# DecodeGenetics/graphtyper

Measured on AMD Instinct MI355X. Metric: aligned+genotyped reads/sec over 1 Mb graph region; VCF bit-identical, higher is better.
Workload: dtype u64/u32 integer (2-bit k-mer keys, byte compares, u32 atomics)

## Files before the change

graphtyper_amd/csrc/gtx_api.hip:

```cpp
#include <hip/hip_runtime.h>
#include <chrono>

#include <algorithm>
#include <cstdio>
#include <cstdlib>
#include <cstring>
#include <memory>
#include <string>

#include "gtx_ctx.hpp"

#include <map>
#include "gtx_devmem.hpp"
#include "gtx_switches.hpp"
#include "wave_hip.hpp"
#include "align_core.hpp"
#include "gtx_hbm_passes.hpp"
#include "score_core.hpp"
#include "score_replay.hpp"

namespace gtx
{
#ifdef GTX_PROF
constexpr uint64_t PROF_LOG_ENTRIES = 1u << 16, PROF_LOG_ENTRY = 16;
// ... 225 lines not shown
    gtx_read_meta next_meta = meta[base];
    for (uint32_t read = base; read < end; ++read)
    {
      gtx_read_meta const m = next_meta;
      if (read + 1 < end)
        next_meta = meta[read + 1];
      uint32_t const len = m.l_qseq;
      uint8_t const * read_seq = seq + static_cast<uint64_t>(read) * seq_stride;
      if (prefetch)
      {
        if (4 * lane < seq_stride)
          seq_words[lane] = next_word;
        WaveHip::lds_sync();
        if (read + 1 < end && 4 * lane < seq_stride)
          next_word = reinterpret_cast<uint32_t const *>(read_seq + seq_stride)[lane];
        read_seq = reinterpret_cast<uint8_t const *>(seq_words);
      }
      bool const too_short = len < 2 * K - 1, too_long = len > AlignCfg::MAX_READ;
      bool const rev = needs_reverse(m, force_both != 0);
      for (uint32_t orient = 0; orient < 2; ++orient)
      {
        uint32_t * rec = records + (static_cast<uint64_t>(read) * 2 + orient) * rec_words;
        if (too_short || too_long || (orient == 1 && !rev))
        {
          if (lane == 0)
          {
            rec[0] = too_long ? (static_cast<uint32_t>(GTX_ST_RECORD_OVERFLOW) << 16) : 0u;
            rec[1] = len << 16;
          }
          continue;
        }
        if (queue_all || !express_one<WaveHip>(g, ix, ws, read_seq, len, orient == 1, rec, rec_words))
        {
          if (lane == 0)
            pending[n_pending] = read * 2 + orient;
          ++n_pending;
        }
      }
    }
    if (n_pending)
    {
      WaveHip::lds_sync();
      uint32_t const at = wave_claim(queue_count, n_pending);
      for (uint32_t k = lane; k < n_pending; k += 64)
        queue[at + k] = pending[k];
      WaveHip::lds_sync();
    }
  }
#ifdef GTX_PROF
  WaveHip::lds_sync();
  if (threadIdx.x < 16)
    atomicAdd(g.prof + threadIdx.x, ws.prof_acc[threadIdx.x]);
#endif
}

template <class E4>
__device__ __forceinline__ void express4_pass(GraphView const & g, IndexView const & ix, uint8_t const * __restrict__ seq, uint32_t seq_stride,
                                              gtx_read_meta const * __restrict__ meta, uint32_t n_reads, uint32_t * __restrict__ records,
                                              uint32_t rec_words, uint32_t force_both, uint32_t * task_counter,
                                              uint32_t * __restrict__ queue, uint32_t * queue_count, uint32_t queue_all)
{
  __shared__ Express4Workspace<E4> ws;
  __shared__ uint8_t pending[2 * TASK_CHUNK];
  static_assert(2 * TASK_CHUNK <= 256, "pending[] holds task offsets as bytes");
  uint32_t const lane = threadIdx.x & 63u;
  for (;;)
  {
    uint32_t const base = wave_claim(task_counter, TASK_CHUNK);
    if (base >= n_reads)
      break;
    uint32_t const end = base + TASK_CHUNK < n_reads ? base + TASK_CHUNK : n_reads;
    uint32_t n_pending = 0;
    for (uint32_t first = base; first < end; first += 4)
    {
      uint32_t const n_valid = end - first < 4 ? end - first : 4;
      uint32_t const gi = lane >> 4;
      bool rev = false;
      if (gi < n_valid)
      {
        gtx_read_meta const m = meta[first + gi];
        uint32_t const len = m.l_qseq;
        rev = needs_reverse(m, force_both != 0) && len >= 2 * K - 1 && len <= AlignCfg::MAX_READ;
        if (!rev && (lane & 15u) == 0)
        {
          uint32_t * rec = records + (static_cast<uint64_t>(first + gi) * 2 + 1) * rec_words;
          rec[0] = len > AlignCfg::MAX_READ ? (static_cast<uint32_t>(GTX_ST_RECORD_OVERFLOW) << 16) : 0u;
          rec[1] = len << 16;
        }
      }
      unsigned long long const REV = __ballot(rev);
      uint32_t const fwd_mask = express4<WaveHip, E4>(g, ix, ws, seq, seq_stride, meta, first, n_valid, records, rec_words, queue_all != 0);
      for (uint32_t k = 0; k < n_valid; ++k)
      {
        if ((fwd_mask >> k) & 1u)
        {
          if (lane == 0)
            pending[n_pending] = static_cast<uint8_t>((first + k - base) * 2);
          ++n_pending;
        }
        if ((REV >> (16 * k)) & 1ull)
        {
          if (lane == 0)
            pending[n_pending] = static_cast<uint8_t>((first + k - base) * 2 + 1);
          ++n_pending;
        }
      }
    }
    if (n_pending)
    {
      WaveHip::lds_sync();
      uint32_t const at = wave_claim(queue_count, n_pending);
      for (uint32_t k = lane; k < n_pending; k += 64)
        queue[at + k] = base * 2 + pending[k];
      WaveHip::lds_sync();
    }
  }
}

#define GTX_EXPRESS4_ARGS                                                                                                          \
  GraphView g, IndexView ix, uint8_t const *__restrict__ seq, uint32_t seq_stride, gtx_read_meta const *__restrict__ meta,         \
    uint32_t n_reads, uint32_t *__restrict__ records, uint32_t rec_words, uint32_t force_both, uint32_t *task_counter,             \
    uint32_t *__restrict__ queue, uint32_t *queue_count, uint32_t queue_all

#ifndef GTX_LEAN_WAVES
#define GTX_LEAN_WAVES 4
#endif
__global__ __launch_bounds__(64) __attribute__((amdgpu_waves_per_eu(GTX_LEAN_WAVES))) void gtx_align_express4_kernel(GTX_EXPRESS4_ARGS)
{
  express4_pass<Express4Lean>(g, ix, seq, seq_stride, meta, n_reads, records, rec_words, force_both, task_counter, queue, queue_count,
                              queue_all);
}

#ifndef GTX_WIDE_WAVES
#define GTX_WIDE_WAVES 4
#endif
__global__ __launch_bounds__(64) __attribute__((amdgpu_waves_per_eu(GTX_WIDE_WAVES))) void gtx_align_express4_wide_kernel(GTX_EXPRESS4_ARGS)
{
  express4_pass<Express4Wide>(g, ix, seq, seq_stride, meta, n_reads, records, rec_words, force_both, task_counter, queue, queue_count,
                              queue_all);
}

template <uint32_t WAVES, bool DENSE, uint32_t NK = AlignCfg::KC, bool META_LDS = true>
__device__ __forceinline__ void hinted_pass(GraphView const & g, IndexView const & ix, uint8_t const * __restrict__ seq, uint32_t seq_stride,
                                            gtx_read_meta const * __restrict__ meta, uint32_t n_reads, uint32_t * __restrict__ records,
                                            uint32_t rec_words, uint32_t force_both, uint32_t * __restrict__ queue1, uint32_t * __restrict__ queue2,
                                            unsigned long long * queue_counts ,
                                            uint32_t decline_all, uint8_t * __restrict__ task_flags, uint32_t * __restrict__ compact,
                                            unsigned long long * __restrict__ var_mask)
{
  constexpr uint32_t ROW_BYTES = HintGeom<NK>::ROW_BYTES, ROW_VEC = ROW_BYTES / 16, META_WORDS = sizeof(gtx_read_meta) / 4;
  constexpr uint32_t ROW_PITCH = NK == AlignCfg::KC ? ROW_VEC : ROW_VEC + 1;
  __shared__ uint4_t s_seq[WAVES][64 * ROW_PITCH];
  __shared__ uint32_t s_meta[META_LDS ? WAVES : 1][META_LDS ? 64 * META_WORDS : 1];
  auto s_count = [&](uint32_t q, uint32_t w) -> uint32_t & { return reinterpret_cast<uint32_t *>(&s_seq[w][0])[q]; };
  auto s_base = [&](uint32_t q) -> uint32_t & { return reinterpret_cast<uint32_t *>(&s_seq[0][0])[2 + q]; };
  static_assert(sizeof(gtx_read_meta) % 4 == 0, "meta records are staged word-wise");
  uint32_t const lane = threadIdx.x & 63u, wave = threadIdx.x >> 6;
  uint32_t const wave_first = blockIdx.x * blockDim.x + wave * 64u;
  uint32_t const read = wave_first + lane;
  bool const full = wave_first + 64u <= n_reads;
  bool const staged = full && seq_stride == ROW_BYTES && (reinterpret_cast<uintptr_t>(seq) & 15u) == 0;
  uint32_t own_meta[META_WORDS] = {};
  if constexpr (META_LDS)
  {
    if (full)
    {
      uint32_t const * src = reinterpret_cast<uint32_t const *>(meta + wave_first);
#pragma unroll
      for (uint32_t it = 0; it < META_WORDS; ++it)
        s_meta[wave][it * 64 + lane] = stream_load(src + it * 64 + lane);
    }
  }
  else if (read < n_reads)
  {
    uint32_t const * src = reinterpret_cast<uint32_t const *>(meta + read);
#pragma unroll
    for (uint32_t it = 0; it < META_WORDS; ++it)
      own_meta[it] = stream_load(src + it);
  }
  if (staged)
  {
    uint4_t const * src = reinterpret_cast<uint4_t const *>(seq + static_cast<uint64_t>(wave_first) * ROW_BYTES);
#pragma unroll
    for (uint32_t it = 0; it < ROW_VEC; ++it)
    {
      uint32_t const v = it * 64 + lane;
      s_seq[wave][ROW_PITCH == ROW_VEC ? v : (v / ROW_VEC) * ROW_PITCH + v % ROW_VEC] = stream_load(src + v);
    }
  }
  else if (read < n_reads)
  {
    uint8_t const * src = seq + static_cast<uint64_t>(read) * seq_stride;
    uint8_t * dst = reinterpret_cast<uint8_t *>(&s_seq[wave][lane * ROW_PITCH]);
#pragma unroll 1
    for (uint32_t k = 0; k < ROW_BYTES; ++k)
      dst[k] = k < seq_stride ? src[k] : static_cast<uint8_t>(0);
  }
  WaveHip::lds_sync();
  bool fwd = false, fwd2 = false, rev = false, staged_rec = false;
  uint32_t fwd_flag = 0;
  bool const compact_wave = compact != nullptr && task_flags != nullptr && full;
  static_assert(HINT_STAGE_WORDS == 16 && HINT_STAGE_WORDS * 4 <= ROW_BYTES, "a staged record is four 16-byte parts inside the read's row");
  if (read < n_reads)
  {
    gtx_read_meta m;
    if constexpr (!META_LDS)
    {
      uint32_t * mw = reinterpret_cast<uint32_t *>(&m);
#pragma unroll
      for (uint32_t k = 0; k < META_WORDS; ++k)
        mw[k] = own_meta[k];
    }
    else if (full)
    {
      uint32_t * mw = reinterpret_cast<uint32_t *>(&m);
#pragma unroll
      for (uint32_t k = 0; k < META_WORDS; ++k)
        mw[k] = s_meta[wave][lane * META_WORDS + k];
    }
    else
      m = meta[read];
    uint32_t const len = m.l_qseq;
    auto rec_at = [&]() -> uint32_t *
    {
      uint32_t r = read;
      GTX_PIN(r);
      return records + static_cast<uint64_t>(r) * 2 * rec_words;
    };
    bool const outside = len < 2 * K - 1 || len > AlignCfg::MAX_READ;
    rev = !outside && needs_reverse(m, force_both != 0);
    if (!rev && (m.flag & GTX_FLAG_FORWARD_ONLY) == 0)
    {
      uint32_t const h0 = len > AlignCfg::MAX_READ ? (static_cast<uint32_t>(GTX_ST_RECORD_OVERFLOW) << 16) : 0u;
      uint32_t * const rec = rec_at();
      if ((rec_words & 1u) == 0 && (reinterpret_cast<uintptr_t>(records) & 7u) == 0)
        *reinterpret_cast<uint2_t *>(rec + rec_words) = uint2_t{h0, len << 16};
      else
      {
        rec[rec_words] = h0;
        rec[rec_words + 1] = len << 16;
      }
    }
    if (outside)
    {
      uint32_t * const rec = rec_at();
      rec[0] = len > AlignCfg::MAX_READ ? (static_cast<uint32_t>(GTX_ST_RECORD_OVERFLOW) << 16) : 0u;
      rec[1] = len << 16;
    }
    else if ((decline_all & 1u) != 0)
      fwd = true;
    else
    {
      uint32_t * row = reinterpret_cast<uint32_t *>(&s_seq[wave][lane * ROW_PITCH]);
      bool const can_stage = (rec_words & 3u) == 0 && (reinterpret_cast<uintptr_t>(records) & 15u) == 0;
      uint32_t where;
      if constexpr (NK == AlignCfg::KC)
        where = hinted_one<DENSE>(g, ix, row, ROW_BYTES, m, rec_at, rec_words, can_stage ? row : nullptr);
      else
        where = hinted_long_one<NK>(g, ix, row, ROW_BYTES, m, rec_at(), rec_words, can_stage ? row : nullptr);
      fwd = where == 0;
      fwd2 = where == HINT_TO_GENERAL;
      staged_rec = where == 2;
      fwd_flag = (where == 0 || where == HINT_TO_GENERAL) ? 0u : ((where == 2 ? row[1] : rec_at()[1]) >> 31);
      if (compact_wave && staged_rec && (row[0] & 0xFFFFu) <= 1u && fwd_flag == 0)
      {
        staged_rec = false;
        fwd_flag = GTX_TASK_COMPACT;
      }
    }
    if ((decline_all & 4u) != 0 && fwd)
    {
      fwd = false;
      fwd2 = true;
    }
    if (task_flags)
    {
      bool const set_fwd = !fwd && !fwd2, set_rev = !rev;
      if (set_fwd && set_rev && (reinterpret_cast<uintptr_t>(task_flags) & 1u) == 0)
        *reinterpret_cast<uint16_t *>(task_flags + 2ull * read) = static_cast<uint16_t>(fwd_flag & 0xFFu);
      else
      {
        if (set_fwd)
          task_flags[2ull * read] = static_cast<uint8_t>(fwd_flag);
        if (set_rev)
          task_flags[2ull * read + 1] = 0;
      }
    }
  }
  if (var_mask)
  {
    unsigned long long const V = __ballot(read < n_reads && !fwd && !fwd2 && (fwd_flag & GTX_TASK_HAS_VARIANTS) != 0u);
    if (lane == 0 && wave_first < n_reads)
      var_mask[wave_first >> 6] = V;
  }
  if (compact_wave)
  {
    WaveHip::lds_sync();
    uint4_t * dst = reinterpret_cast<uint4_t *>(compact + static_cast<uint64_t>(wave_first) * GTX_COMPACT_WORDS);
#pragma unroll
    for (uint32_t k = 0; k < 2; ++k)
    {
      uint32_t const r = 32u * k + (lane >> 1);
      stream_store(dst + 64u * k + lane, s_seq[wave][r * ROW_PITCH + (lane & 1u)]);
    }
  }
  {
    unsigned long long const S = __ballot(staged_rec);
    if (S != 0)
    {
      uint32_t const part = lane & 3u;
#pragma unroll
      for (uint32_t round = 0; round < 4; ++round)
      {
        uint32_t const r = round * 16u + (lane >> 2);
        if ((S >> r) & 1ull)
        {
          uint4_t const v = s_seq[wave][r * ROW_PITCH + part];
          uint32_t const rd = wave_first + r;
          uint32_t * dst = records + static_cast<uint64_t>(rd) * 2 * rec_words;
          stream_store(reinterpret_cast<uint4_t *>(dst + 4 * part), v);
        }
      }
    }
  }
  unsigned long long const F = __ballot(fwd), R = __ballot(rev), F2 = __ballot(fwd2);
  if (lane == 0)
  {
    s_count(0, wave) = static_cast<uint32_t>(__builtin_popcountll(F));
    s_count(1, wave) = static_cast<uint32_t>(__builtin_popcountll(R) + __builtin_popcountll(F2));
  }
  __syncthreads();
  if (threadIdx.x == 0)
  {
    uint32_t total1 = 0, total2 = 0;
    for (uint32_t w = 0; w < WAVES; ++w)
    {
      total1 += s_count(0, w);
      total2 += s_count(1, w);
    }
    unsigned long long base = 0;
    if (total1 | total2)
      base = atomicAdd(queue_counts, (static_cast<unsigned long long>(total1) << 32) | total2);
    s_base(0) = static_cast<uint32_t>(base >> 32);
    s_base(1) = static_cast<uint32_t>(base);
  }
  __syncthreads();
  uint32_t off1 = s_base(0), off2 = s_base(1);
  for (uint32_t w = 0; w < WAVES; ++w)
    if (w < wave)
    {
      off1 += s_count(0, w);
      off2 += s_count(1, w);
    }
  if (fwd)
    queue1[off1 + static_cast<uint32_t>(__builtin_popcountll(F & ((1ull << lane) - 1ull)))] = read;
  if (rev)
    queue2[off2 + static_cast<uint32_t>(__builtin_popcountll(R & ((1ull << lane) - 1ull)))] = read * 2 + 1;
  if (fwd2)
    queue2[off2 + static_cast<uint32_t>(__builtin_popcountll(R) + __builtin_popcountll(F2 & ((1ull << lane) - 1ull)))] = read * 2;
}

#define GTX_HINTED_ARGS                                                                                                            \
  GraphView g, IndexView ix, uint8_t const *__restrict__ seq, uint32_t seq_stride, gtx_read_meta const *__restrict__ meta,         \
    uint32_t n_reads, uint32_t *__restrict__ records, uint32_t rec_words, uint32_t force_both, uint32_t *__restrict__ queue1,      \
    uint32_t *__restrict__ queue2, unsigned long long *queue_counts, uint32_t decline_all, uint8_t *__restrict__ task_flags,       \
    uint32_t *__restrict__ compact, unsigned long long *span, unsigned long long *__restrict__ var_mask
#define GTX_HINTED_PASS(W, ...)                                                                                                    \
  if (span && threadIdx.x == 0 && blockIdx.x == 0)                                                                                 \
    atomicMax(span, ~static_cast<unsigned long long>(wall_clock64()));                                                             \
  hinted_pass<W, __VA_ARGS__>(g, ix, seq, seq_stride, meta, n_reads, records, rec_words, force_both, queue1, queue2, queue_counts, decline_all, task_flags, compact, var_mask); \
  if (span && threadIdx.x == 0 && blockIdx.x + 1024u >= gridDim.x && ((blockIdx.x & 15u) == 15u || blockIdx.x + 1u == gridDim.x))   \
    atomicMax(span + 1, static_cast<unsigned long long>(wall_clock64()))

#ifndef GTX_HINT_VGPRS
#define GTX_HINT_VGPRS 72
#endif
#ifndef GTX_HINT_WAVES
#define GTX_HINT_WAVES 1
#endif
#ifndef GTX_HINT_PER_EU
#define GTX_HINT_PER_EU 7
#endif
#ifndef GTX_HINT_WAVES_LEAN
#define GTX_HINT_WAVES_LEAN 2
#endif
__global__ __launch_bounds__(64 * GTX_HINT_WAVES_LEAN) __attribute__((amdgpu_num_vgpr(GTX_HINT_VGPRS), amdgpu_waves_per_eu(GTX_HINT_PER_EU, GTX_HINT_PER_EU))) void gtx_align_hinted_kernel(GTX_HINTED_ARGS)
{
  GTX_HINTED_PASS(GTX_HINT_WAVES_LEAN, false, AlignCfg::KC, GTX_HINT_PER_EU <= 6);
}

#ifndef GTX_HINT_DENSE_WAVES
#define GTX_HINT_DENSE_WAVES 4
#endif
__global__ __launch_bounds__(64 * GTX_HINT_WAVES) __attribute__((amdgpu_waves_per_eu(GTX_HINT_DENSE_WAVES, GTX_HINT_DENSE_WAVES))) void gtx_align_hinted_dense_kernel(GTX_HINTED_ARGS)
{
  GTX_HINTED_PASS(GTX_HINT_WAVES, true);
}

__global__ __launch_bounds__(64 * GTX_HINT_WAVES) __attribute__((amdgpu_waves_per_eu(3, 3))) void gtx_align_hinted_long_kernel(GTX_HINTED_ARGS)
{
  GTX_HINTED_PASS(GTX_HINT_WAVES, false, 8);
}

constexpr uint32_t EXPRESS_GROUPS_PER_WAVE = 4, GENERAL_TASKS_PER_WAVE = 3;
template <class E4>
__device__ __forceinline__ void express4_queue_pass(GraphView const & g, IndexView const & ix, uint8_t const * __restrict__ seq,
                                                    uint32_t seq_stride, gtx_read_meta const * __restrict__ meta,
                                                    uint32_t * __restrict__ records, uint32_t rec_words, uint32_t * task_counter,
                                                    uint32_t const * __restrict__ queue1, uint32_t const * queue1_count,
                                                    uint32_t * __restrict__ queue2, uint32_t * queue2_count, uint32_t * handed_on,
                                                    uint32_t queue_all)
{
  __shared__ Express4Workspace<E4> ws;
  __shared__ uint32_t pending[TASK_CHUNK];
  uint32_t const lane = threadIdx.x & 63u;
  uint32_t const n = queue1_count[0];
  uint32_t const n_groups = (n + 3u) / 4u, G_all = gridDim.x;
  uint32_t const per_wave_goal = (queue_all >> 8) ? (queue_all >> 8) : EXPRESS_GROUPS_PER_WAVE;
  uint32_t const G_want = (n_groups + per_wave_goal - 1u) / per_wave_goal;
  uint32_t const G = G_want >= G_all ? G_all : G_want > 0u ? G_want : 1u;
  if (blockIdx.x >= G)
    return;
  uint32_t const own = n_groups / G <= 8u ? (n_groups / G) * 3u / 4u : 0u;
#ifdef GTX_PROF
  if (threadIdx.x < 16)
    ws.prof_acc[threadIdx.x] = 0;
  WaveHip::lds_sync();
#endif
  uint32_t n_pending = 0;
  auto flush = [&]()
  {
    if (n_pending)
    {
      WaveHip::lds_sync();
      uint32_t const at = wave_claim(queue2_count, n_pending);
      if (lane == 0)
        atomicAdd(handed_on, n_pending);
      for (uint32_t k = lane; k < n_pending; k += 64)
        queue2[at + k] = pending[k];
      WaveHip::lds_sync();
      n_pending = 0;
    }
  };
  uint32_t const per_visit = n_groups / G >= 128u ? 16u : n_groups / G >= 32u ? 4u : 1u;
  for (uint32_t i = 0, grp = 0, grp_end = 0;; ++i, ++grp)
  {
    if (i < own)
      grp = blockIdx.x + i * G;
    else if (i == own || grp == grp_end)
    {
      grp = own * G + wave_claim(task_counter, per_visit);
      grp_end = grp + per_visit;
    }
    if (grp >= n_groups)
      break;
    uint32_t const first = 4u * grp;
    uint32_t const n_valid = n - first < 4 ? n - first : 4;
    uint32_t const fwd_mask = express4<WaveHip, E4>(g, ix, ws, seq, seq_stride, meta, 0, n_valid, records, rec_words, (queue_all & 1u) != 0, queue1 + first);
    for (uint32_t k = 0; k < n_valid; ++k)
      if ((fwd_mask >> k) & 1u)
      {
        if (lane == 0)
          pending[n_pending] = queue1[first + k] * 2;
        ++n_pending;
      }
    if (n_pending + 4u > TASK_CHUNK)
      flush();
  }
  flush();
#ifdef GTX_PROF
  WaveHip::lds_sync();
  if (threadIdx.x < 16)
    atomicAdd(g.prof + 16 + threadIdx.x, ws.prof_acc[threadIdx.x]);
#endif
}

#define GTX_EXPRESS4Q_ARGS                                                                                                         \
  GraphView g, IndexView ix, uint8_t const *__restrict__ seq, uint32_t seq_stride, gtx_read_meta const *__restrict__ meta,         \
    uint32_t *__restrict__ records, uint32_t rec_words, uint32_t *task_counter, uint32_t const *__restrict__ queue1,               \
    uint32_t const *queue1_count, uint32_t *__restrict__ queue2, uint32_t *queue2_count, uint32_t *handed_on, uint32_t queue_all

__global__ __launch_bounds__(64) __attribute__((amdgpu_waves_per_eu(GTX_LEAN_WAVES))) void gtx_align_express4q_kernel(GTX_EXPRESS4Q_ARGS)
{
  express4_queue_pass<Express4Lean>(g, ix, seq, seq_stride, meta, records, rec_words, task_counter, queue1, queue1_count, queue2,
                                    queue2_count, handed_on, queue_all);
}

__global__ __launch_bounds__(64) __attribute__((amdgpu_waves_per_eu(GTX_WIDE_WAVES))) void gtx_align_express4q_wide_kernel(GTX_EXPRESS4Q_ARGS)
{
  express4_queue_pass<Express4Wide>(g, ix, seq, seq_stride, meta, records, rec_words, task_counter, queue1, queue1_count, queue2,
                                    queue2_count, handed_on, queue_all);
}

#ifndef GTX_GENERAL_WAVES
#define GTX_GENERAL_WAVES 5
#endif
__global__ __launch_bounds__(64) __attribute__((amdgpu_waves_per_eu(GTX_GENERAL_WAVES))) void gtx_align_kernel(GraphView g, IndexView ix, uint8_t const * __restrict__ seq,
                                                       uint32_t seq_stride, gtx_read_meta const * __restrict__ meta,
                                                       uint32_t * __restrict__ records, uint32_t rec_words,
                                                       uint32_t const * __restrict__ queue, uint32_t const * queue_count,
                                                       uint32_t * task_counter, uint32_t * __restrict__ big_tasks,
                                                       uint32_t big_task_cap, uint32_t * big_state, uint32_t force_big, uint32_t task_base,
                                                       uint32_t claim, uint32_t * forward_done)
{
  __shared__ AlignWorkspace ws;
#ifdef GTX_PROF
  if (threadIdx.x < 16)
    ws.prof_acc[threadIdx.x] = 0;
  WaveHip::lds_sync();
#endif
  uint32_t const queued = queue_count[0];
  uint32_t const per_wave_goal = (force_big >> 8) ? (force_big >> 8) : GENERAL_TASKS_PER_WAVE;
// ... 2282 lines not shown
```

graphtyper_amd/csrc/hinted.hpp:

```cpp
#pragma once
#include <type_traits>

#include "graph_dev.hpp"

namespace gtx
{
#ifdef GTX_EMU_NOTES
void hint_note(uint32_t code);
#define GTX_HINT_NOTE(code) hint_note(code)
#else
#define GTX_HINT_NOTE(code) ((void)0)
#endif

constexpr uint32_t HINT_MAX_READ = 160;
constexpr uint32_t HINT_WORDS = HINT_MAX_READ / 8;

GTX_DEV uint32_t hint_bswap(uint32_t v)
{
  return __builtin_bswap32(v);
}

GTX_DEV uint32_t nib_nonzero(uint32_t v)
{
  v |= v >> 1;
// ... 855 lines not shown
        {
          best = xa;
          mask = 0;
        }
        if (xa == best)
          mask |= 1u << a;
      }
    x0 = ((codes & 15u) != rc && rc != 15u) ? 1u : 0u;
    return best;
  };
  auto carried = [&](uint32_t km, uint32_t site) -> uint32_t
  {
    uint32_t set = (km >> HK_SET_SHIFT) & 255u;
    if (DENSE && hk_is_two(km))
    {
      uint32_t const s0 = km >> HK_SITE_SHIFT;
      if (site != s0 && site != s0 + 1u)
        return 4u;
      set = site == s0 ? (set & 15u) : (set >> 4);
      return (set & (set - 1u)) != 0 ? 4u : static_cast<uint32_t>(__builtin_ctz(set));
    }
    if ((km >> HK_SITE_SHIFT) != site || (set & (set - 1u)) != 0)
      return 4u;
    return set ? static_cast<uint32_t>(__builtin_ctz(set)) : (km >> HK_ALLELE_SHIFT) & 3u;
  };
  uint32_t head_site = 0, head_mask = 0;
  if (prs != 0 && !decided)
  {
    uint32_t const y = lo == 1 ? f1.y : lo == 2 ? f2.y : lo == 3 ? f3.y : f4.y;
    uint32_t const back = (y >> HINT_BACK_SHIFT) & 255u;
    uint32_t upto = hc_upto(h, lo) + hc_edge(h, lo);
    if ((y & 255u) == 0 || back < prs)
    {
      bool const on_site = (y & 255u) == 0;
      uint32_t const ps = on_site ? prs : prs - back - 1u;
      if (idx + ps == 0)
      {
        GTX_HINT_NOTE(11);
        return false;
      }
      uint32_t const q = idx + ps - 1u;
      uint32_t const yq = ix.pos_flags[q].y;
      uint2_t const tq = ix.tail_info[q];
      uint32_t const km = lo == 1 ? k1 : lo == 2 ? k2 : lo == 3 ? k3 : k4;
      uint32_t const only = on_site ? carried(km, tq.y) : 4u;
      if ((yq & 255u) != 1u || (tq.x & HINT_TAIL_OK) == 0 || (ps != 0 && ((yq >> HINT_BACK_SHIFT) & 255u) + 1u < ps) || (on_site && only >= 4u))
      {
        GTX_HINT_NOTE(11);
        return false;
      }
      uint32_t mask = 0, x0 = 0;
      uint32_t const best = site_choice(tq.x, plane_code_at(row, ps), only, mask, x0);
      upto = upto - x0 + best;
      head_site = tq.y;
      head_mask = mask;
    }
    uint32_t const head_len = prs + 1;
    uint32_t const budget = 2 + head_len / 11 < 7 ? 2 + head_len / 11 : 7;
    if (upto <= budget)
    {
      start = order_of(idx);
      rs = 0;
      mism += upto;
    }
    else
      head_mask = 0;
  }
  uint32_t end = order_of(idx + pre), re = pre;
  uint32_t tail_site = 0, tail_mask = 0;
  uint32_t tail_mask2 = 0;
  if (decided)
  {
    start = order_of(idx + two_rs);
    rs = two_rs;
    re = two_re;
    end = order_of(idx + two_re);
    mism = two_mism;
  }
  else if (pre != L - 1)
  {
    uint32_t const tail_len = L - pre;
    uint32_t const budget = 2 + tail_len / 11 < 7 ? 2 + tail_len / 11 : 7;
    uint32_t tail_end = DENSE ? order_of(idx + L - 1u) : 0u;
    uint32_t const y = hi + 1 == n_k ? y_end : hi == 0 ? f1.y : hi == 1 ? f2.y : hi == 2 ? f3.y : f4.y;
    uint32_t const room = y & 255u;
    uint32_t got = hc_all(h) - hc_upto(h, hi + 1);
    if (room < tail_len)
    {
      bool const on_site = room == 0;
      uint32_t const at = room;
      uint2_t ti = t_end;
      uint32_t only = 4u;
      bool ok = true;
      if (on_site)
      {
        uint32_t const q = idx + pre - 1u;
        ok = (ix.pos_flags[q].y & 255u) == 1u;
        ti = ix.tail_info[q];
        only = carried(hi == 0 ? k0 : hi == 1 ? k1 : hi == 2 ? k2 : hi == 3 ? k3 : k4, ti.y);
        ok = ok && only < 4u;
      }
      else if (hi + 1 != n_k)
        ti = ix.tail_info[idx + pre];
      uint32_t const next_len = (ti.x >> HINT_TAIL_NEXT_SHIFT) & 255u;
      if (!ok || (ti.x & HINT_TAIL_OK) == 0 || next_len < tail_len - at - 1)
      {
        bool walked = false;
        if constexpr (DENSE)
          if (!on_site && (ti.x & HINT_TAIL_NODE) != 0 && tail_len <= 64)
          {
            HintWalk const w = hint_tail_walk(g, ix, row, idx, pre, tail_len, at, ti.y, budget);
            if (w.status == 2)
            {
              GTX_HINT_NOTE(8);
              return HINT_TO_GENERAL;
            }
            if (w.status == 1)
            {
              walked = true;
              got = w.got;
              tail_end = w.end;
              tail_site = ti.y;
              tail_mask = w.mask1;
              tail_mask2 = w.mask2;
            }
          }
        if (!walked)
        {
          GTX_HINT_NOTE(8);
          return false;
        }
      }
      else
      {
        uint32_t mask = 0, x0 = 0;
        uint32_t const best = site_choice(ti.x, plane_code_at(row, pre + at), only, mask, x0);
        got = got - x0 + best;
        tail_site = ti.y;
        tail_mask = mask;
      }
    }
    if (got <= budget)
    {
      re = L - 1;
      mism += got;
      if constexpr (DENSE)
        end = tail_end;
      else
        end += tail_len - 1;
    }
    else
      tail_mask = tail_mask2 = 0;
  }
  uint32_t v0 = 0, v1 = 0, v2 = 0, v3 = 0, v4 = 0, v5 = 0;
  uint32_t nvar = 0;
  uint32_t last = 0xFFFFFFFFu;
  bool clash = false;
  auto append = [&](uint32_t entry)
  {
    if constexpr (DENSE)
    {
      bool found = false;
      auto meet = [&](uint32_t & v, uint32_t at)
      {
        if (at < nvar && (v >> 16) == (entry >> 16))
        {
          v &= entry | 0xFFFF0000u;
          clash = clash || (v & 0xFFFFu) == 0;
          found = true;
        }
      };
      meet(v0, 0);
      meet(v1, 1);
      meet(v2, 2);
      meet(v3, 3);
      meet(v4, 4);
      meet(v5, 5);
      if (!found)
      {
        v0 = nvar == 0 ? entry : v0;
        v1 = nvar == 1 ? entry : v1;
        v2 = nvar == 2 ? entry : v2;
        v3 = nvar == 3 ? entry : v3;
        v4 = nvar == 4 ? entry : v4;
        v5 = nvar == 5 ? entry : v5;
        ++nvar;
      }
    }
    else if ((entry >> 16) == (last >> 16))
    {
      last &= entry | 0xFFFF0000u;
      clash = clash || (last & 0xFFFFu) == 0;
      v0 = nvar == 1 ? last : v0;
      v1 = nvar == 2 ? last : v1;
      v2 = nvar == 3 ? last : v2;
      v3 = nvar == 4 ? last : v3;
      v4 = nvar == 5 ? last : v4;
      v5 = nvar == 6 ? last : v5;
    }
    else
    {
      v0 = nvar == 0 ? entry : v0;
      v1 = nvar == 1 ? entry : v1;
      v2 = nvar == 2 ? entry : v2;
      v3 = nvar == 3 ? entry : v3;
      v4 = nvar == 4 ? entry : v4;
      v5 = nvar == 5 ? entry : v5;
      ++nvar;
      last = entry;
    }
  };
  auto push = [&](uint32_t k, uint32_t km)
  {
    if (((run >> k) & 1u) && (km >> HK_SITE_SHIFT) != HINT_NO_SITE)
    {
      uint32_t const set = (km >> HK_SET_SHIFT) & 255u;
      if (DENSE && hk_is_two(km))
      {
        append(((km >> HK_SITE_SHIFT) << 16) | (set & 15u));
        append((((km >> HK_SITE_SHIFT) + 1u) << 16) | (set >> 4));
      }
      else
        append(((km >> HK_SITE_SHIFT) << 16) | (set ? set : 1u << ((km >> HK_ALLELE_SHIFT) & 3u)));
    }
  };
  if (tail_mask != 0)
    append((tail_site << 16) | tail_mask);
  if (tail_mask2 != 0)
    append(((tail_site + 1u) << 16) | tail_mask2);
  push(4, k4);
  push(3, k3);
  push(2, k2);
  push(1, k1);
  push(0, k0);
  if (head_mask != 0)
    append((head_site << 16) | head_mask);
  if (clash || nvar > 6 || 6 + 3 * nvar > rec_words)
  {
    GTX_HINT_NOTE(13);
    return false;
  }
  uint32_t np = 1, longest = re - rs + 1;
  if (par_start && rs == 0)
  {
    uint32_t const amb_lo = hc_get(lo == 1 ? h.k[1] : lo == 2 ? h.k[2] : lo == 3 ? h.k[3] : h.k[4], HC_AMB);
    uint2_t const f_lo = lo == 1 ? f1 : lo == 2 ? f2 : lo == 3 ? f3 : f4;
    bool two_chains = amb_lo != 0;
    if (!two_chains)
    {
      uint32_t const off = (f_lo.y >> HINT_SNPOFF_SHIFT) & 31u;
      if ((f_lo.x & HINT_ALT_OK) == 0 || off == K - 1)
      {
        GTX_HINT_NOTE(106);
        return HINT_TO_GENERAL;
      }
      two_chains = off != 0;
    }
    if (two_chains)
    {
      uint32_t const mm_run = mmk & run, km_hi = hi == 0 ? k0 : hi == 1 ? k1 : hi == 2 ? k2 : hi == 3 ? k3 : k4;
      auto plain = [&](uint32_t k, uint32_t km) { return ((run >> k) & 1u) == 0 || (km & ((3u << HK_ALLELE_SHIFT) | (255u << HK_SET_SHIFT))) == 0; };
      uint32_t alt_sites = 0;
      uint32_t const other = (plain(0, k0) ? 0u : 1u) | (plain(1, k1) ? 0u : 2u) | (plain(2, k2) ? 0u : 4u) | (plain(3, k3) ? 0u : 8u) | (plain(4, k4) ? 0u : 16u);
      if (other != 0)
      {
        uint32_t const k = static_cast<uint32_t>(__builtin_ctz(other));
        uint32_t const km = k == 0 ? k0 : k == 1 ? k1 : k == 2 ? k2 : k == 3 ? k3 : k4;
        uint32_t const yk = ix.pos_flags[idx + (K - 1) * k].y;
        bool ok = ix.hint_less == 0 && mm_run == 0 && pw == nullptr;
        ok = ok && (other & (other - 1u)) == 0 && ((km >> HK_SET_SHIFT) & 255u) == 0;
        alt_sites = (K - 1) * k + ((yk >> HINT_SNPOFF_SHIFT) & 31u) < pre ? 1u : 0u;
        if (!ok)
        {
          GTX_HINT_NOTE(107);
          return HINT_TO_GENERAL;
        }
      }
      bool const region_clean = hc_upto(h, hi + 1) == hc_upto(h, lo) + alt_sites;
      if (mm_run == (1u << hi) && hi + 1 > 4)
      {
        GTX_HINT_NOTE(108);
        return HINT_TO_GENERAL;
      }
      bool const last_only = mm_run == (1u << hi) && hc_edge(h, hi + 1) == 1 && ((km_hi >> HK_SET_SHIFT) & 255u) == 0;
      bool const twin = region_clean && (mm_run == 0 || last_only);
      if (pre == L - 1 || re != L - 1 || (twin && nvar > 1))
      {
        GTX_HINT_NOTE(109);
        return HINT_TO_GENERAL;
      }
      if (twin && mm_run == 0)
        np = 2;
      else if (twin)
        --mism;
    }
  }
  if (mism > 10)
  {
    np = 0;
    longest = 0;
  }
  uint32_t const path_words = 4 + 3 * nvar;
  if (2 + np * path_words > rec_words)
    return false;
  bool const to_stage = stage != nullptr && rec_words >= HINT_STAGE_WORDS && 2 + (np ? np : 1u) * path_words <= HINT_STAGE_WORDS;
  uint32_t * rec = to_stage ? stage : hint_rec_ptr(rec_at);
  if (to_stage)
  {
#pragma unroll
    for (uint32_t k = 2; k < HINT_STAGE_WORDS; ++k)
      rec[k] = 0u;
  }
  rec[0] = np;
  rec[1] = longest | (L << 16) | ((np && nvar) ? GTX_REC_HAS_VARIANTS : 0u);
  if (np)
  {
    rec[2] = start;
    rec[3] = end;
    rec[4] = rs | (re << 16);
    rec[5] = mism | (nvar << 16);
    auto put = [&](uint32_t k, uint32_t entry)
    {
      if (k < nvar)
      {
        rec[6 + 3 * k] = entry >> 16;
        rec[7 + 3 * k] = entry & 0xFFFFu;
        rec[8 + 3 * k] = 0u;
      }
    };
    put(0, v0);
    put(1, v1);
    put(2, v2);
    put(3, v3);
    put(4, v4);
    put(5, v5);
    if (np == 2)
      for (uint32_t k = 0; k < path_words; ++k)
        rec[2 + path_words + k] = rec[2 + k];
  }
  return to_stage ? 2u : 1u;
}

template <bool DENSE, class Row, class Rec>
GTX_DEV uint32_t hinted_one(GraphView const & g, IndexView const & ix, Row row, uint32_t seq_stride, gtx_read_meta const & m,
                            Rec rec, uint32_t rec_words, uint32_t * stage = nullptr)
{
  uint32_t const L = m.l_qseq;
  if (L < 2 * K - 1 || L > HINT_MAX_READ || m.pos < 0 || ix.n_hint == 0)
  {
    GTX_HINT_NOTE(9);
    return false;
  }
  if (static_cast<uint32_t>(m.pos) < ix.hint_first)
    return false;
  uint32_t const idx = static_cast<uint32_t>(m.pos) - ix.hint_first;
  if (idx >= ix.n_hint || L > ix.n_hint - idx)
    return false;
  uint32_t mm_main = 0xFFFFu;
  uint32_t where = hinted_on_path<DENSE>(g, ix, row, seq_stride, m, idx, static_cast<HintWindow const *>(nullptr), 0u, rec, rec_words, stage, mm_main);
  if constexpr (DENSE)
  {
    if (where == 0 && ix.n_win != 0 && mm_main != 0xFFFFu)
    {
      uint2_t const t0 = ix.tail_info[idx];
      if ((t0.x & HINT_TAIL_NODE) != 0)
      {
        uint32_t best = mm_main, best_at = 0, best_w = INVALID, tried = 0;
        uint32_t r = t0.y;
#pragma unroll 1
        for (uint32_t s = 0; s < 4 && r + 1 < g.n_ref; ++s, ++r)
        {
          uint32_t const off = g.ref_order[r] + g.ref_len[r] - (g.first_order + idx);
          if (off >= L)
            break;
          uint32_t const sw = ix.site_win[r], first = sw & 0xFFFFFFu, count = sw >> 24;
#pragma unroll 1
          for (uint32_t k = 0; k < count && tried < 8; ++k, ++tried)
          {
            uint32_t const at = ix.win_base + (first + k) * HINT_WIN_STRIDE + (HINT_WIN_BEFORE - off);
            uint32_t const mm = hint_mm_linear(row, ix.refp, 0u, at, L);
            if (mm < best)
            {
              best = mm;
              best_at = at;
              best_w = first + k;
            }
          }
        }
        if (best_w != INVALID)
        {
          uint32_t mm_w = 0;
          where = hinted_on_path<DENSE>(g, ix, row, seq_stride, m, best_at, ix.win + best_w, ix.win_base + best_w * HINT_WIN_STRIDE, rec, rec_words, stage, mm_w);
        }
      }
    }
  }
  return where;
}

}
```

Before: 19.18 billion.

## Use per-wave queue atomics, compact staged-record flush, and stream variant entries directly

Result: faster. 19.43 billion (median of 6 runs) (+1.3%).

```diff
diff --git a/graphtyper_amd/csrc/gtx_api.hip b/graphtyper_amd/csrc/gtx_api.hip
--- a/graphtyper_amd/csrc/gtx_api.hip
+++ b/graphtyper_amd/csrc/gtx_api.hip
@@ -401,8 +401,6 @@
   constexpr uint32_t ROW_PITCH = NK == AlignCfg::KC ? ROW_VEC : ROW_VEC + 1;
   __shared__ uint4_t s_seq[WAVES][64 * ROW_PITCH];
   __shared__ uint32_t s_meta[META_LDS ? WAVES : 1][META_LDS ? 64 * META_WORDS : 1];
-  auto s_count = [&](uint32_t q, uint32_t w) -> uint32_t & { return reinterpret_cast<uint32_t *>(&s_seq[w][0])[q]; };
-  auto s_base = [&](uint32_t q) -> uint32_t & { return reinterpret_cast<uint32_t *>(&s_seq[0][0])[2 + q]; };
   static_assert(sizeof(gtx_read_meta) % 4 == 0, "meta records are staged word-wise");
   uint32_t const lane = threadIdx.x & 63u, wave = threadIdx.x >> 6;
   uint32_t const wave_first = blockIdx.x * blockDim.x + wave * 64u;
@@ -449,7 +447,8 @@
   bool fwd = false, fwd2 = false, rev = false, staged_rec = false;
   uint32_t fwd_flag = 0;
   bool const compact_wave = compact != nullptr && task_flags != nullptr && full;
-  static_assert(HINT_STAGE_WORDS == 16 && HINT_STAGE_WORDS * 4 <= ROW_BYTES, "a staged record is four 16-byte parts inside the read's row");
+  static_assert(HINT_STAGE_WORDS == 16 && (HINT_STAGE_WORDS + 4) * 4 <= ROW_BYTES,
+                "a staged record is four 16-byte parts inside the read's row, with four spare words behind it");
   if (read < n_reads)
   {
     gtx_read_meta m;
@@ -558,12 +557,18 @@
     if (S != 0)
     {
       uint32_t const part = lane & 3u;
-#pragma unroll
-      for (uint32_t round = 0; round < 4; ++round)
+      uint32_t const n_staged = static_cast<uint32_t>(__builtin_popcountll(S));
+      uint32_t * const rows = reinterpret_cast<uint32_t *>(&s_seq[wave][0]);
+      if (staged_rec)
+        rows[static_cast<uint32_t>(__builtin_popcountll(S & ((1ull << lane) - 1ull))) * (ROW_PITCH * 4u) + HINT_STAGE_WORDS] = lane;
+      WaveHip::lds_sync();
+#pragma unroll 1
+      for (uint32_t first = 0; first < n_staged; first += 16u)
       {
-        uint32_t const r = round * 16u + (lane >> 2);
-        if ((S >> r) & 1ull)
+        uint32_t const j = first + (lane >> 2);
+        if (j < n_staged)
         {
+          uint32_t const r = rows[j * (ROW_PITCH * 4u) + HINT_STAGE_WORDS];
           uint4_t const v = s_seq[wave][r * ROW_PITCH + part];
           uint32_t const rd = wave_first + r;
           uint32_t * dst = records + static_cast<uint64_t>(rd) * 2 * rec_words;
@@ -573,40 +578,21 @@
     }
   }
   unsigned long long const F = __ballot(fwd), R = __ballot(rev), F2 = __ballot(fwd2);
+  if ((F | R | F2) == 0)
+    return;
+  uint32_t const n_rev = static_cast<uint32_t>(__builtin_popcountll(R));
+  unsigned long long base = 0;
   if (lane == 0)
-  {
-    s_count(0, wave) = static_cast<uint32_t>(__builtin_popcountll(F));
-    s_count(1, wave) = static_cast<uint32_t>(__builtin_popcountll(R) + __builtin_popcountll(F2));
-  }
-  __syncthreads();
-  if (threadIdx.x == 0)
-  {
-    uint32_t total1 = 0, total2 = 0;
-    for (uint32_t w = 0; w < WAVES; ++w)
-    {
-      total1 += s_count(0, w);
-      total2 += s_count(1, w);
-    }
-    unsigned long long base = 0;
-    if (total1 | total2)
-      base = atomicAdd(queue_counts, (static_cast<unsigned long long>(total1) << 32) | total2);
-    s_base(0) = static_cast<uint32_t>(base >> 32);
-    s_base(1) = static_cast<uint32_t>(base);
-  }
-  __syncthreads();
-  uint32_t off1 = s_base(0), off2 = s_base(1);
-  for (uint32_t w = 0; w < WAVES; ++w)
-    if (w < wave)
-    {
-      off1 += s_count(0, w);
-      off2 += s_count(1, w);
-    }
+    base = atomicAdd(queue_counts, (static_cast<unsigned long long>(__builtin_popcountll(F)) << 32) |
+                                     (n_rev + static_cast<uint32_t>(__builtin_popcountll(F2))));
+  uint32_t const off1 = __builtin_amdgcn_readfirstlane(static_cast<uint32_t>(base >> 32));
+  uint32_t const off2 = __builtin_amdgcn_readfirstlane(static_cast<uint32_t>(base));
   if (fwd)
     queue1[off1 + static_cast<uint32_t>(__builtin_popcountll(F & ((1ull << lane) - 1ull)))] = read;
   if (rev)
     queue2[off2 + static_cast<uint32_t>(__builtin_popcountll(R & ((1ull << lane) - 1ull)))] = read * 2 + 1;
   if (fwd2)
-    queue2[off2 + static_cast<uint32_t>(__builtin_popcountll(R) + __builtin_popcountll(F2 & ((1ull << lane) - 1ull)))] = read * 2;
+    queue2[off2 + n_rev + static_cast<uint32_t>(__builtin_popcountll(F2 & ((1ull << lane) - 1ull)))] = read * 2;
 }
 
 #define GTX_HINTED_ARGS                                                                                                            \
diff --git a/graphtyper_amd/csrc/hinted.hpp b/graphtyper_amd/csrc/hinted.hpp
--- a/graphtyper_amd/csrc/hinted.hpp
+++ b/graphtyper_amd/csrc/hinted.hpp
@@ -1031,10 +1031,49 @@
     else
       tail_mask = tail_mask2 = 0;
   }
+  bool const to_row = stage != nullptr && rec_words >= HINT_STAGE_WORDS;
   uint32_t v0 = 0, v1 = 0, v2 = 0, v3 = 0, v4 = 0, v5 = 0;
   uint32_t nvar = 0;
   uint32_t last = 0xFFFFFFFFu;
   bool clash = false;
+  if constexpr (!DENSE)
+    if (to_row)
+    {
+#pragma unroll
+      for (uint32_t k = 2; k < HINT_STAGE_WORDS; ++k)
+        stage[k] = 0u;
+    }
+  auto entry_out = [&](uint32_t k, uint32_t entry)
+  {
+    if (to_row)
+    {
+      if (k < 4)
+      {
+        stage[6 + 3 * k] = entry >> 16;
+        stage[7 + 3 * k] = entry & 0xFFFFu;
+      }
+      else if (k < 6)
+        stage[HINT_STAGE_WORDS - 2 + k] = entry;
+    }
+    else if (9 + 3 * k <= rec_words)
+    {
+      uint32_t * const slot = hint_rec_ptr(rec_at);
+      slot[6 + 3 * k] = entry >> 16;
+      slot[7 + 3 * k] = entry & 0xFFFFu;
+      slot[8 + 3 * k] = 0u;
+    }
+  };
+  auto entries_back = [&]()
+  {
+    if constexpr (!DENSE)
+      if (!to_row && nvar != 0)
+      {
+        uint32_t * const slot = hint_rec_ptr(rec_at);
+#pragma unroll 1
+        for (uint32_t k = 6; k + 3 <= rec_words && k < 6 + 3 * nvar; k += 3)
+          slot[k] = slot[k + 1] = slot[k + 2] = 0u;
+      }
+  };
   auto append = [&](uint32_t entry)
   {
     if constexpr (DENSE)
@@ -1070,21 +1109,11 @@
     {
       last &= entry | 0xFFFF0000u;
       clash = clash || (last & 0xFFFFu) == 0;
-      v0 = nvar == 1 ? last : v0;
-      v1 = nvar == 2 ? last : v1;
-      v2 = nvar == 3 ? last : v2;
-      v3 = nvar == 4 ? last : v3;
-      v4 = nvar == 5 ? last : v4;
-      v5 = nvar == 6 ? last : v5;
+      entry_out(nvar - 1, last);
     }
     else
     {
-      v0 = nvar == 0 ? entry : v0;
-      v1 = nvar == 1 ? entry : v1;
-      v2 = nvar == 2 ? entry : v2;
-      v3 = nvar == 3 ? entry : v3;
-      v4 = nvar == 4 ? entry : v4;
-      v5 = nvar == 5 ? entry : v5;
+      entry_out(nvar, entry);
       ++nvar;
       last = entry;
     }
@@ -1117,6 +1146,7 @@
   if (clash || nvar > 6 || 6 + 3 * nvar > rec_words)
   {
     GTX_HINT_NOTE(13);
+    entries_back();
     return false;
   }
   uint32_t np = 1, longest = re - rs + 1;
@@ -1131,6 +1161,7 @@
       if ((f_lo.x & HINT_ALT_OK) == 0 || off == K - 1)
       {
         GTX_HINT_NOTE(106);
+        entries_back();
         return HINT_TO_GENERAL;
       }
       two_chains = off != 0;
@@ -1152,6 +1183,7 @@
         if (!ok)
         {
           GTX_HINT_NOTE(107);
+          entries_back();
           return HINT_TO_GENERAL;
         }
       }
@@ -1159,6 +1191,7 @@
       if (mm_run == (1u << hi) && hi + 1 > 4)
       {
         GTX_HINT_NOTE(108);
+        entries_back();
         return HINT_TO_GENERAL;
       }
       bool const last_only = mm_run == (1u << hi) && hc_edge(h, hi + 1) == 1 && ((km_hi >> HK_SET_SHIFT) & 255u) == 0;
@@ -1166,6 +1199,7 @@
       if (pre == L - 1 || re != L - 1 || (twin && nvar > 1))
       {
         GTX_HINT_NOTE(109);
+        entries_back();
         return HINT_TO_GENERAL;
       }
       if (twin && mm_run == 0)
@@ -1181,41 +1215,82 @@
   }
   uint32_t const path_words = 4 + 3 * nvar;
   if (2 + np * path_words > rec_words)
+  {
+    entries_back();
     return false;
-  bool const to_stage = stage != nullptr && rec_words >= HINT_STAGE_WORDS && 2 + (np ? np : 1u) * path_words <= HINT_STAGE_WORDS;
-  uint32_t * rec = to_stage ? stage : hint_rec_ptr(rec_at);
-  if (to_stage)
-  {
+  }
+  bool const to_stage = to_row && 2 + (np ? np : 1u) * path_words <= HINT_STAGE_WORDS;
+  auto finish = [&](uint32_t * rec)
+  {
+    rec[0] = np;
+    rec[1] = longest | (L << 16) | ((np && nvar) ? GTX_REC_HAS_VARIANTS : 0u);
+    if (np)
+    {
+      rec[2] = start;
+      rec[3] = end;
+      rec[4] = rs | (re << 16);
+      rec[5] = mism | (nvar << 16);
+      if (np == 2)
+        for (uint32_t k = 0; k < path_words; ++k)
+          rec[2 + path_words + k] = rec[2 + k];
+    }
+  };
+  if constexpr (DENSE)
+  {
+    uint32_t * rec = to_stage ? stage : hint_rec_ptr(rec_at);
+    if (to_stage)
+    {
 #pragma unroll
-    for (uint32_t k = 2; k < HINT_STAGE_WORDS; ++k)
-      rec[k] = 0u;
-  }
-  rec[0] = np;
-  rec[1] = longest | (L << 16) | ((np && nvar) ? GTX_REC_HAS_VARIANTS : 0u);
-  if (np)
-  {
-    rec[2] = start;
-    rec[3] = end;
-    rec[4] = rs | (re << 16);
-    rec[5] = mism | (nvar << 16);
-    auto put = [&](uint32_t k, uint32_t entry)
-    {
-      if (k < nvar)
-      {
-        rec[6 + 3 * k] = entry >> 16;
-        rec[7 + 3 * k] = entry & 0xFFFFu;
-        rec[8 + 3 * k] = 0u;
-      }
-    };
-    put(0, v0);
-    put(1, v1);
-    put(2, v2);
-    put(3, v3);
-    put(4, v4);
-    put(5, v5);
-    if (np == 2)
-      for (uint32_t k = 0; k < path_words; ++k)
-        rec[2 + path_words + k] = rec[2 + k];
+      for (uint32_t k = 2; k < HINT_STAGE_WORDS; ++k)
+        rec[k] = 0u;
+    }
+    if (np)
+    {
+      auto put = [&](uint32_t k, uint32_t entry)
+      {
+        if (k < nvar)
+        {
+          rec[6 + 3 * k] = entry >> 16;
+          rec[7 + 3 * k] = entry & 0xFFFFu;
+          rec[8 + 3 * k] = 0u;
+        }
+      };
+      put(0, v0);
+      put(1, v1);
+      put(2, v2);
+      put(3, v3);
+      put(4, v4);
+      put(5, v5);
+    }
+    finish(rec);
+  }
+  else if (to_stage)
+  {
+    if (np == 0 && nvar != 0)
+    {
+#pragma unroll 1
+      for (uint32_t k = 6; k < 6 + 3 * nvar; ++k)
+        stage[k] = 0u;
+    }
+    finish(stage);
+  }
+  else
+  {
+    uint32_t * const slot = hint_rec_ptr(rec_at);
+    if (to_row && np)
+    {
+#pragma unroll 1
+      for (uint32_t k = 0; k < nvar; ++k)
+      {
+        uint32_t const entry = k < 4 ? (stage[6 + 3 * k] << 16) | stage[7 + 3 * k] : stage[HINT_STAGE_WORDS - 2 + k];
+        slot[6 + 3 * k] = entry >> 16;
+        slot[7 + 3 * k] = entry & 0xFFFFu;
+        slot[8 + 3 * k] = 0u;
+      }
+    }
+    if (np == 0)
+      entries_back();
+    finish(slot);
   }
   return to_stage ? 2u : 1u;
 }
```
